# hanyas/mimo

Measured on AMD Instinct MI355X. Metric: E-step datapoint-component evals/sec, higher is better.
Workload: dtype f64

## Files before the change

include/mimo_hip.h:

```cpp
#ifndef MIMO_HIP_H
#define MIMO_HIP_H

#include <stddef.h>
#include <stdint.h>

#ifdef __cplusplus
extern "C" {
#endif

typedef struct mimo_ctx mimo_ctx;

#define MIMO_OK               0
#define MIMO_E_INVALID       -1
#define MIMO_E_HIP           -2
#define MIMO_E_NODATA        -3
#define MIMO_E_UNSUPPORTED   -4
#define MIMO_E_STATE         -5
#define MIMO_E_NOMEM         -6
#define MIMO_E_INTERNAL      -7

#define MIMO_F_KEEP_RESP      0x01
#define MIMO_F_KEEP_LOGP      0x02
#define MIMO_F_KEEP_LSE       0x04
#define MIMO_F_NO_STATS       0x08
// ... 155 lines not shown
                           const double* sx, const double* sn, const double* sxx,
                           double* alpha, double* qa, double* qb, double* qc, double* qd,
                           double* mus, double* psis, double* nus, double* half_logdet_psi, double* nat_c,
                           double* cc, double* bb, double* W, double* E2, double* E4, double* e_log_pi, double* c_total);
int mimo_host_gmm_vi_bound(int K, int D, int tied, const double* alpha0, const double* alpha, const double* e_log_pi,
                           const double* pa, const double* pb, const double* pc, const double* pd, const double* prior_logZ,
                           const double* qa, const double* qb, const double* qc, const double* qd,
                           const double* mus, const double* nus, const double* half_logdet_psi, const double* nat_c,
                           const double* bb, const double* E2, const double* W, const double* E4, double* vlb);

int mimo_host_block_order(int K, int D, const double* means, const double* mass, int block, int32_t* order);

int mimo_host_estep_certificate(int K, int D, const double* c0, const double* b0, const double* W0, const double* c, const double* b,
                                const double* W, double margin, double* out, double* table);

int mimo_host_legacy_draws(uint32_t* mt_key, int* mt_pos, int* has_gauss, double* gauss, int K, int n_before,
                           int n_gamma, int n_after, const double* shapes, double* before, double* gammas,
                           double* after);

int mimo_host_hier_vi(int K, int D, int nb_iter, const double* kap, const double* m0, double kappa0, const double* psi0_inv,
                      double nu0, const double* xk, const double* nk, const double* sxx_sum, double* mu_q, double* post_mus,
                      double* post_kappas, double* kappa_q, double* psi_q, double* nu_q);

int mimo_host_legacy_draws_inplace(uint32_t* mt_key, int* mt_pos, int has_gauss, double gauss, int K, int n_before,
                                   int n_gamma, int n_after, const double* shapes, double* before, double* gammas,
                                   double* after, int* redraw, uint32_t* final_state);

int mimo_host_py_sample(uint32_t* mt_key, int* mt_pos, int64_t n, int64_t k, int use_pool, int64_t* out);

int mimo_host_mnw_vi(int K, int dy, int dc, int affine, const double* a, const double* b, const double* c,
// ... 51 lines not shown
```

mimo_amd/_lib.py:

```python
import ctypes as C
import os
import sys

_HERE = os.path.dirname(os.path.abspath(__file__))
LIB_PATH = os.environ.get("MIMO_HIP_LIB") or os.path.join(_HERE, "libmimo_hip.so")

OK = 0
E_INVALID, E_HIP, E_NODATA, E_UNSUPPORTED, E_STATE, E_NOMEM, E_INTERNAL = -1, -2, -3, -4, -5, -6, -7
F_KEEP_RESP, F_KEEP_LOGP, F_KEEP_LSE, F_NO_STATS, F_DEVICE_OUT, F_DEVICE_IN, F_ENTROPY_SPLIT, F_ASYNC = 1, 2, 4, 8, 0x10, 0x20, 0x40, 0x80
F_WEIGHTS_RESIDENT = 0x100
F_DIAG_VAR = 0x200
F_SVI_RESIDENT_START = 0x400

_dp = C.POINTER(C.c_double)
_ip = C.POINTER(C.c_int32)
_vp = C.c_void_p

SIGNATURES = {
    "mimo_create": (C.c_int, [C.POINTER(_vp), C.c_int]),
    "mimo_destroy": (C.c_int, [_vp]),
    "mimo_last_error": (C.c_char_p, [_vp]),
    "mimo_set_stream": (C.c_int, [_vp, _vp]),
    "mimo_upload": (C.c_int, [_vp, _vp, C.c_int64, C.c_int]),
    "mimo_attach": (C.c_int, [_vp, _vp, C.c_int64, C.c_int]),
# ... 33 lines not shown
    "mimo_sample_from_log": (C.c_int, [_vp, _vp, C.c_int, C.c_int64, _vp, C.c_uint64, C.c_uint64, C.c_int, _vp, _vp]),
    "mimo_random_resp_stats": (C.c_int, [_vp, C.c_int, C.c_uint64, C.c_int, _vp]),
    "mimo_host_nw_vi": (C.c_int, [C.c_int, C.c_int] + [_vp] * 13),
    "mimo_host_nw_vi_tied": (C.c_int, [C.c_int, C.c_int] + [_vp] * 14),
    "mimo_host_nw_vlb": (C.c_int, [C.c_int, C.c_int] + [_vp] * 16),
    "mimo_host_legacy_draws_inplace": (C.c_int, [_vp, _vp, C.c_int, C.c_double, C.c_int, C.c_int, C.c_int, C.c_int,
                                                 _vp, _vp, _vp, _vp, C.POINTER(C.c_int), _vp]),
    "mimo_host_py_sample": (C.c_int, [_vp, C.POINTER(C.c_int), C.c_int64, C.c_int64, C.c_int, _vp]),
    "mimo_host_hier_vi": (C.c_int, [C.c_int, C.c_int, C.c_int, _vp, _vp, C.c_double, _vp, C.c_double] + [_vp] * 9),
    "mimo_host_legacy_draws": (C.c_int, [_vp, C.POINTER(C.c_int), C.POINTER(C.c_int), C.POINTER(C.c_double),
                                         C.c_int, C.c_int, C.c_int, C.c_int, _vp, _vp, _vp, _vp]),
    "mimo_host_gmm_vi_sweep": (C.c_int, [C.c_int, C.c_int, C.c_int] + [_vp] * 26),
    "mimo_host_gmm_vi_bound": (C.c_int, [C.c_int, C.c_int, C.c_int] + [_vp] * 21),
    "mimo_host_block_order": (C.c_int, [C.c_int, C.c_int, _vp, _vp, C.c_int, _vp]),
    "mimo_host_estep_certificate": (C.c_int, [C.c_int, C.c_int, _vp, _vp, _vp, _vp, _vp, _vp, C.c_double, _vp, _vp]),
    "mimo_host_mnw_vi": (C.c_int, [C.c_int, C.c_int, C.c_int, C.c_int] + [_vp] * 15),
    "mimo_host_nw_gibbs": (C.c_int, [C.c_int, C.c_int] + [_vp] * 10),
    "mimo_host_digamma": (C.c_double, [C.c_double]),
    "mimo_host_checksum": (C.c_int, [_vp, C.c_size_t, C.POINTER(C.c_uint64)]),
    "mimo_predict": (C.c_int, [_vp, _vp, _vp, _vp, C.c_int, _vp, _vp, _vp, C.c_int, C.c_int, C.c_int,
                               _vp, _vp, _vp, _vp, _vp, _vp]),
    "mimo_predict_flags": (C.c_int, [_vp, _vp, _vp, _vp, C.c_int, _vp, _vp, _vp, C.c_int, C.c_int, C.c_int,
                                     _vp, _vp, _vp, _vp, _vp, _vp, C.c_int]),
    "mimo_predict_batched": (C.c_int, [_vp, C.c_int, _vp, _vp, C.c_int64, C.c_int, _vp, _vp, _vp, _vp, C.c_int,
                                       _vp, _vp, _vp, C.c_int, C.c_int, _vp, _vp, _vp, _vp, _vp, _vp, _vp, C.c_int]),
    "mimo_get_resp": (C.c_int, [_vp, _vp]),
    "mimo_get_resp_columns": (C.c_int, [_vp, _vp, C.c_int64, _vp]),
    "mimo_get_logp": (C.c_int, [_vp, _vp]),
    "mimo_get_lse": (C.c_int, [_vp, _vp]),
    "mimo_get_labels": (C.c_int, [_vp, _vp]),
# ... 48 lines not shown
```

mimo_amd/csrc/mimo_abi.cpp:

```cpp
#include "mimo_abi_internal.h"
#include "mimo_kernels.h"
#include "mimo_extra.h"
#include "mimo_route.h"

#include <algorithm>
#include <cmath>
#include <cstdarg>
#include <cstdio>
#include <cstdlib>
#include <cstring>
#include <limits>
#include <new>
#include <stdexcept>
#include <string>
#include <vector>

using namespace mimo;
using namespace mimo_abi;

namespace mimo_comm {
int unique_id(char* out128, char* msg, size_t msglen);
int init(void** comm, const char* id128, int rank, int world, char* msg, size_t msglen);
int destroy(void* comm);
int allreduce_sum_f64(void* comm, double* buf, size_t count, hipStream_t stream, char* msg, size_t msglen);
// ... 109 lines not shown

static constexpr int kCertRenew = 16;
static constexpr double kCertEps = 1e-3;
static int cert_plan(mimo_ctx* ctx, const KernelArgs& a, const double* c, const double* b, const double* W, double* tab, int* kind) {
  *kind = kCertNone;
  const int K = a.K, D = ctx->D;
  if (!ctx->cert_on || a.resp_skip <= 0 || a.K16 != 4 || D < 14 || D > kMaxFusedD || ctx->structure != 0 || ctx->N < 1) return MIMO_OK;
  uint64_t part[4] = {0, 0, 0, 0};
  int32_t slot_of[64];
  for (int s = 0; s < K; ++s) { part[s >> 4] |= 1ull << ctx->order[s]; slot_of[ctx->order[s]] = s; }
  std::sort(part, part + 4);
  const bool stood = ctx->cert_prev_K == K && !memcmp(part, ctx->cert_prev_part, sizeof part);
  memcpy(ctx->cert_prev_part, part, sizeof part);
  ctx->cert_prev_K = K;
  if (ctx->cert_valid && (ctx->cert_K != K || ctx->cert_skip != a.resp_skip || memcmp(part, ctx->cert_part, sizeof part))) ctx->cert_valid = false;
  const size_t KD = (size_t)K * D, KDD = KD * D;
  if (ctx->cert_valid && ctx->cert_age < kCertRenew) {
    double out[5 * 64 + 4], t[4 + 2 * 64];
    const double* r = ctx->cert_ref.data();
    if (mimo_host_estep_certificate(K, D, r, r + K, r + K + KD, c, b, W, -0.6931471805599453 * a.resp_skip - kCertEps, out, t) == MIMO_OK) {
      memcpy(tab, t, 4 * sizeof(double));
      uint8_t* blk = reinterpret_cast<uint8_t*>(tab + 4 + 128);
      for (int s = 0; s < 64; ++s) {
        const int k = s < K ? ctx->cert_order[s] : -1;
        tab[4 + s] = k < 0 ? -1e300 : t[4 + k];
        tab[4 + 64 + s] = k < 0 ? 0.0 : t[4 + K + k];
        blk[s] = k < 0 ? 0 : (uint8_t)(slot_of[k] >> 4);
      }
      ctx->cert_age += 1;
      *kind = kCertCertified;
      return MIMO_OK;
    }
    ctx->cert_valid = false;
  }
  if (!stood) return MIMO_OK;
  int rc;
  if ((rc = ctx->cert_k.ensure(ctx, (size_t)ctx->N)) || (rc = ctx->cert_m.ensure(ctx, (size_t)ctx->N)) || (rc = ctx->cert_a.ensure(ctx, (size_t)ctx->N))) return rc;
  if (!ctx->cert_cnt.p) {
    if ((rc = ctx->cert_cnt.ensure(ctx, 4))) return rc;
    HIP_TRY(ctx, hipMemsetAsync(ctx->cert_cnt, 0, 4 * sizeof(unsigned long long), ctx->stream));
  }
  ctx->cert_ref.resize(K + KD + KDD);
  memcpy(ctx->cert_ref.data(), c, K * sizeof(double));
  memcpy(ctx->cert_ref.data() + K, b, KD * sizeof(double));
  memcpy(ctx->cert_ref.data() + K + KD, W, KDD * sizeof(double));
  memcpy(ctx->cert_order, ctx->order, K * sizeof(int32_t));
  memcpy(ctx->cert_part, part, sizeof part);
  ctx->cert_K = K; ctx->cert_skip = a.resp_skip; ctx->cert_age = 0;
  ctx->cert_valid = true;
  *kind = kCertReference;
  return MIMO_OK;
}

static void fill_args(mimo_ctx* ctx, int K, KernelArgs* a) {
  memset(a, 0, sizeof *a);
  a->Z = ctx->Z; a->N = ctx->N; a->D = ctx->D; a->K = K; a->K16 = (K + 15) / 16;
  a->F16 = ctx->F16;
  a->ZS = route_zs(K, ctx->D);
  a->RS = ctx->F16 + rs_pad();
  a->F16_total = ctx->F16;
// ... 1200 lines not shown
```

mimo_amd/csrc/mimo_host.cpp:

```cpp
#include <algorithm>
#include <atomic>
#include <condition_variable>
#include <functional>
#include <mutex>
#include <cmath>
#include <pthread.h>
#include <cstdint>
#include <cstdlib>
#include <cstring>
#include <new>
#include <stdexcept>
#include <system_error>
#include <thread>
#include <vector>

#include "../../include/mimo_hip.h"

namespace {

constexpr double kLog2Pi = 1.8378770664093454835606594728112;
constexpr double kLog2 = 0.69314718055994530941723212145818;

double digamma(double x) {
  double r = 0.0;
  while (x < 10.0) { r -= 1.0 / x; x += 1.0; }
  const double f = 1.0 / (x * x);
  const double t = f * (-1.0 / 12.0 + f * (1.0 / 120.0 + f * (-1.0 / 252.0 + f * (1.0 / 240.0 + f * (-1.0 / 132.0
                   + f * (691.0 / 32760.0 + f * (-1.0 / 12.0)))))));
// ... 967 lines not shown
    for (int i = c; i < A; ++i) {
      if (find(i) != c) continue;
      put(b >= 0 ? b : lightest(1), i);
    }
  }
  int s = 0;
  for (int k = 0; k < K; ++k) {
    if (mass[k] >= 1.0) continue;
    while (order[s] >= 0) ++s;
    order[s] = k;
  }
  return MIMO_OK;
  });
}

namespace {
constexpr double kCertGrid[] = {0.98, 0.95, 0.9, 0.8, 0.65, 0.5, 0.3, 0.1};

unsigned cert_chol4(v4d* __restrict__ M, int n) {
  unsigned bad = 0;
  v4d d0[32];
  for (int j = 0; j < n; ++j) d0[j] = M[j * n + j];
  for (int j = 0; j < n; ++j) {
    v4d* mj = M + (size_t)j * n;
    v4d d = mj[j], piv;
    for (int l = 0; l < 4; ++l) {
      if (!(d[l] > 1e-10 * std::fabs(d0[j][l]))) { bad |= 1u << l; d[l] = 1.0; }
      piv[l] = std::sqrt(d[l]);
    }
    const v4d inv = 1.0 / piv;
    for (int c = j; c < n; ++c) mj[c] *= inv;
    for (int i = j + 1; i < n; ++i) {
      const v4d f = mj[i];
      v4d* mi = M + (size_t)i * n;
      for (int c = i; c < n; ++c) mi[c] -= f * mj[c];
    }
  }
  return bad;
}
}

int mimo_host_estep_certificate(int K, int D, const double* c0, const double* b0, const double* W0, const double* c, const double* b,
                                const double* W, double margin, double* out, double* table) {
  return guarded_host([&]() -> int {
  if (K < 1 || D < 1 || !c0 || !b0 || !W0 || !c || !b || !W || !out) return MIMO_E_INVALID;
  if (K > 256 || D > 32) return MIMO_E_UNSUPPORTED;
  const size_t DD = (size_t)D * D;
  for (size_t i = 0; i < (size_t)K; ++i) if (!std::isfinite(c0[i]) || !std::isfinite(c[i])) return MIMO_E_INVALID;
  for (size_t i = 0; i < (size_t)K * D; ++i) if (!std::isfinite(b0[i]) || !std::isfinite(b[i])) return MIMO_E_INVALID;
  for (size_t i = 0; i < (size_t)K * DD; ++i) if (!std::isfinite(W0[i]) || !std::isfinite(W[i])) return MIMO_E_INVALID;
  double *ch0 = out, *ch = out + K, *rho = out + 2 * (size_t)K, *rhob = out + 3 * (size_t)K, *dk = out + 4 * (size_t)K, *cons = out + 5 * (size_t)K;
  std::vector<v4d> work(5 * DD);
  v4d *A0 = work.data(), *A1 = A0 + DD, *U0 = A1 + DD, *U1 = U0 + DD, *T = U1 + DD;
  v4d y[32], mu0[32], mu1[32];
  auto solve = [&](const v4d* U, const double* const rhs[4], v4d* mu) {
    v4d yy = {0.0, 0.0, 0.0, 0.0};
    for (int i = 0; i < D; ++i) {
      v4d s = {rhs[0][i], rhs[1][i], rhs[2][i], rhs[3][i]};
      for (int r = 0; r < i; ++r) s -= U[r * D + i] * y[r];
      y[i] = s / U[i * D + i];
      yy += y[i] * y[i];
    }
    for (int i = D - 1; i >= 0; --i) {
      v4d s = y[i];
      for (int r = i + 1; r < D; ++r) s -= U[i * D + r] * mu[r];
      mu[i] = s / U[i * D + i];
    }
    return yy;
  };
  for (int k0 = 0; k0 < K; k0 += 4) {
    int kk[4];
    for (int l = 0; l < 4; ++l) kk[l] = std::min(k0 + l, K - 1);
    const double *a0[4], *a1[4], *r0[4], *r1[4];
    for (int l = 0; l < 4; ++l) { a0[l] = W0 + kk[l] * DD; a1[l] = W + kk[l] * DD; r0[l] = b0 + (size_t)kk[l] * D; r1[l] = b + (size_t)kk[l] * D; }
    for (int i = 0; i < D; ++i)
      for (int j = i; j < D; ++j) {
        const size_t e = (size_t)i * D + j;
        U0[e] = A0[e] = v4d{a0[0][e], a0[1][e], a0[2][e], a0[3][e]};
        U1[e] = A1[e] = v4d{a1[0][e], a1[1][e], a1[2][e], a1[3][e]};
      }
    if (cert_chol4(U0, D) | cert_chol4(U1, D)) return MIMO_E_INVALID;
    const v4d q0 = solve(U0, r0, mu0), q1 = solve(U1, r1, mu1);
    v4d d2 = {0.0, 0.0, 0.0, 0.0};
    for (int i = 0; i < D; ++i) {
      v4d s = {0.0, 0.0, 0.0, 0.0};
      for (int r = i; r < D; ++r) s += U0[i * D + r] * (mu1[r] - mu0[r]);
      d2 += s * s;
    }
    unsigned same = 0;
    for (int l = 0; l < 4; ++l) if (!memcmp(a0[l], a1[l], DD * sizeof(double))) same |= 1u << l;
    double lo[4] = {0.0, 0.0, 0.0, 0.0}, hi[4] = {HUGE_VAL, HUGE_VAL, HUGE_VAL, HUGE_VAL};
    for (int side = 0; side < 2; ++side) {
      const v4d *P = side ? A0 : A1, *Q = side ? A1 : A0;
      unsigned pending = 0xFu & ~same;
      for (const double s : kCertGrid) {
        if (!pending) break;
        for (int i = 0; i < D; ++i)
          for (int j = i; j < D; ++j) T[i * D + j] = P[i * D + j] - s * Q[i * D + j];
        const unsigned ok = pending & ~cert_chol4(T, D);
        for (int l = 0; l < 4; ++l) if (ok >> l & 1u) { if (side) hi[l] = 1.0 / s; else lo[l] = s; }
        pending &= ~ok;
      }
    }
    for (int l = 0; l < 4 && k0 + l < K; ++l) {
      const int k = k0 + l;
      ch0[k] = c0[k] + 0.5 * q0[l];
      ch[k] = c[k] + 0.5 * q1[l];
      dk[k] = std::sqrt(d2[l]);
      rho[k] = (same >> l & 1u) ? 1.0 : lo[l];
      rhob[k] = (same >> l & 1u) ? 1.0 : hi[l];
    }
  }
  cons[0] = ch0[0]; cons[1] = ch[0]; cons[2] = rho[0]; cons[3] = dk[0];
  for (int k = 1; k < K; ++k) {
    cons[0] = std::min(cons[0], ch0[k]); cons[1] = std::max(cons[1], ch[k]);
    cons[2] = std::min(cons[2], rho[k]); cons[3] = std::max(cons[3], dk[k]);
  }
  if (!table) return MIMO_OK;
  std::vector<double> srt(ch0, ch0 + K);
  std::sort(srt.begin(), srt.end());
  double cut = HUGE_VAL, widest = 0.0;
// ... 11 lines not shown
    const double beta = rmin * (1.0 - e);
    table[2 * cl] = cmax - beta * c0min + 0.5 * rmin * (1.0 / e - 1.0) * dmax * dmax;
    table[2 * cl + 1] = beta;
  }
  double *gam = table + 4, *del = table + 4 + K;
  for (int k = 0; k < K; ++k) {
    if (!(rhob[k] < HUGE_VAL)) { gam[k] = -1e300; del[k] = 0.0; continue; }
    const double e = std::min(std::max(dk[k], 1e-12) / 4.0, 1.0);
    del[k] = rhob[k] * (1.0 + e);
    gam[k] = ch[k] - del[k] * ch0[k] - 0.5 * rhob[k] * (1.0 + 1.0 / e) * dk[k] * dk[k] + margin;
  }
  return MIMO_OK;
  });
}

double mimo_host_digamma(double x) { return digamma(x); }

int mimo_host_debug_fault(int kind) {
  return guarded_host([&]() -> int {
    if (kind == 1) throw std::bad_alloc();
    if (kind == 2) throw std::runtime_error("mimo_host_debug_fault");
    if (kind == 3) throw 42;
    if (kind == 4) { g_fail_thread_start.store(1); return MIMO_OK; }
    return kind == 0 ? MIMO_OK : MIMO_E_INVALID;
  });
}

}
```

mimo_amd/csrc/mimo_kernels.hip:

```cpp
#include "mimo_tile.h"
#include "mimo_extra.h"
#include <cstdio>
#include <cstdlib>

#include <math.h>
#include <type_traits>
#include <utility>

namespace mimo {

double philox_uniform_host(uint64_t seed, uint64_t row, uint64_t sweep) {
  return philox_uniform(seed, row, sweep);
}

#ifndef MIMO_ASYM_PRIO
#define MIMO_ASYM_PRIO 0
#endif
#define MFMA_PRIO()                                                                        \
  do {                                                                                    \
    if (MIMO_ASYM_PRIO && prio_hi) __builtin_amdgcn_s_setprio(1);                         \
    else __builtin_amdgcn_s_setprio(0);                                                   \
  } while (0)

#ifndef MIMO_STAGGER
// ... 144 lines not shown
    }
  };
  auto store_z = [&](int64_t t) {
#pragma unroll
    for (int i = 0; i < ZPT; ++i)
      if (zoff[i] >= 0) Zs[zoff[i]] = zr[i];
    if (tid < T) {
      if constexpr (TRIM) Zs[tid * ZS + D] = tid < clamp_scalar(N - t * T, T) ? 1.0 : 0.0;
      else Zs[tid * ZS + D] = (t * T + tid) < N ? 1.0 : 0.0;
      Zs[tid * ZS + D + 1] = 0.0;
    }
  };
  load_z(blockIdx.x);
  store_z(blockIdx.x);
  load_z((int64_t)blockIdx.x + gridDim.x);
  int ck = 0, nk = 0;
  double cm = 0.0, ca = 0.0, nm = 0.0, na = 0.0;
  auto load_cert = [&](int64_t t, int& k, double& m, double& av) {
    const int64_t n = t * T + (lane & 31);
    const bool in = n < N;
    k = in ? (int)a.cert_k[n] & 63 : 0;
    m = in ? a.cert_m[n] : 0.0;
    av = in ? a.cert_a[n] : 0.0;
  };
  double ctab[4] = {0.0, 0.0, 0.0, 0.0};
  double* const ctl = reinterpret_cast<double*>(fe + 2 * F16);
  uint32_t cnt_proven = 0, cnt_one = 0, cnt_all = 0;
  if constexpr (CERT == kCertCertified) {
    load_cert(blockIdx.x, ck, cm, ca);
    load_cert((int64_t)blockIdx.x + gridDim.x, nk, nm, na);
#pragma unroll
    for (int i = 0; i < 4; ++i) ctab[i] = a.cert_tab[i];
    for (int e = tid; e < kCertTabLen - 4; e += kWG) ctl[e] = a.cert_tab[4 + e];
  }

  const int frow = tid & (T - 1), fgrp = tid >> 5;
  wg_sync();
  uint32_t w[NCB];
  if constexpr (DS == 0) {
#pragma unroll
    for (int jj = 0; jj < NCB; ++jj) w[jj] = reinterpret_cast<const uint32_t*>(fe)[fgrp * NCB + jj];
  }

  STAGGER_START();
#ifdef MIMO_STAMPS
  unsigned long long st_sum[8] = {0, 0, 0, 0, 0, 0, 0, 0}, st_prev;
  asm volatile("s_memtime %0\n\ts_waitcnt lgkmcnt(0)" : "=s"(st_prev)::"memory");
#endif
#ifdef MIMO_STAMPS
  int st_it = 0;
#endif
  for (int64_t t = blockIdx.x; t < a.ntiles; t += gridDim.x) {
// ... 52 lines not shown
        const int k = kq + 8 * it;
        if (k < Kpad) Lt[pt * LS + k] = wv[it];
      }
    } else if constexpr (SRC == kSrcLabels) {
      if (tid < T) labs[tid] = (n0 + tid) < N ? a.labels[n0 + tid] : -1;
    }
    STAMP(1);
    MFMA_PRIO();
    wg_sync();
    STAMP(2);
#ifdef MIMO_STAMPS
    if (st_trace) st_tr[1] = st_prev;
#endif

    if constexpr (SRC == kSrcEstep) {
      uint32_t need = 0xFFFFFFFFu, computed = 0xFFFFFFFFu;
      if constexpr (CERT == kCertCertified) {
        const bool in = n0 + (lane & 31) < N;
        const double cgam = ctl[ck], cdel = ctl[64 + ck];
        const int cblk = reinterpret_cast<const uint8_t*>(ctl + 128)[ck];
        const double ub = fmax(fma(ctab[1], ca, ctab[0]), fma(ctab[3], ca, ctab[2]));
        const bool proven = in && ub <= fma(cdel, cm, cgam);
        const uint32_t pm = (uint32_t)__builtin_amdgcn_ballot_w64(proven);
        const uint32_t b0 = (uint32_t)__builtin_amdgcn_ballot_w64((cblk & 1) != 0), b1 = (uint32_t)__builtin_amdgcn_ballot_w64((cblk & 2) != 0);
        uint32_t eff[4];
#pragma unroll
        for (int w = 0; w < 4; ++w) {
          const uint32_t nd = ~pm | (((w & 1) ? b0 : ~b0) & ((w & 2) ? b1 : ~b1));
          eff[w] = __builtin_popcount(nd) <= 16 ? nd : 0xFFFFFFFFu;
        }
        need = wave == 0 ? eff[0] : wave == 1 ? eff[1] : wave == 2 ? eff[2] : eff[3];
        computed = lane < 16 ? eff[0] : lane < 32 ? eff[1] : lane < 48 ? eff[2] : eff[3];
        if (wave == 0) cnt_proven += __builtin_popcount(pm);
        cnt_one += need != 0xFFFFFFFFu ? 1u : 0u;
        cnt_all += 1u;
      }
      if constexpr (is_split) {
        if (sidx < 2) {
          gptr_t th = (gptr_t)(a.theta + (size_t)srb * NSI * 64);
          asm volatile("" : "+s"(th));
          const double* p = Ph + (16 * sidx + j) * RS + q;
          d4 acc = d4{0.0, 0.0, 0.0, 0.0};
          constexpr int PD = NS < 8 ? NS : 8;
          double tr[PD], bq[3];
#pragma unroll
          for (int e = 0; e < PD; ++e) tr[e] = th[e * 64 + lane];
          bq[0] = p[0];
          if (NS > 1) bq[1] = p[4];
#pragma unroll
          for (int s2 = 0; s2 < NS; ++s2) {
            if (s2 + 2 < NS) bq[(s2 + 2) % 3] = p[4 * (s2 + 2)];
// ... 3 lines not shown
            acc = __builtin_amdgcn_mfma_f64_16x16x4f64(av, bq[s2 % 3], acc, 0, 0, 0);
          }
          int lw_off = (16 * sidx + j) * LS + 16 * srb + q;
          asm volatile("" : "+v"(lw_off));
          double* lw = Lt + lw_off;
#pragma unroll
          for (int r = 0; r < 4; ++r) lw[4 * r] = acc[r];
        }
      } else if (wave < K16) {
        thw = thw0;
        asm volatile("" : "+s"(thw));
        if constexpr (SEED_TILE) load_seed(thw);
        const double* p0 = Ph + j * RS + q;
        const double* p1 = Ph + (16 + j) * RS + q;
        bool one_group = false;
        if constexpr (CERT == kCertCertified) one_group = need != 0xFFFFFFFFu;
        if (one_group) {
          if constexpr (CERT == kCertCertified) {
            const int cnt = __builtin_popcount(need);
            int rj = need ? __builtin_ctz(need) : 0;
            {
              uint32_t mleft = need;
              for (int jj = 0; mleft; ++jj) {
                rj = j == jj ? __builtin_ctz(mleft) : rj;
                mleft &= mleft - 1;
              }
            }
            int p_off = rj * RS + q;
            asm volatile("" : "+v"(p_off));
            const double* pc = Ph + p_off;
            d4 acc = SEED ? d4{cseed[0], cseed[1], cseed[2], cseed[3]} : d4{0.0, 0.0, 0.0, 0.0};
            double bq[3];
            bq[0] = pc[0];
            if (NS > 1) bq[1] = pc[4];
#pragma unroll
            for (int s = 0; s < NS; ++s) {
              if (s + 2 < NS) bq[(s + 2) % 3] = pc[4 * (s + 2)];
              __builtin_amdgcn_sched_barrier(0);
              const double av = ring[s % PF];
              ring[s % PF] = theta_slice((s + PF) % NEP);
              acc = __builtin_amdgcn_mfma_f64_16x16x4f64(av, bq[s % 3], acc, 0, 0, 0);
            }
            if (j < cnt) {
              int lw_off = rj * LS + 16 * wave + q;
              asm volatile("" : "+v"(lw_off));
              double* lw = Lt + lw_off;
#pragma unroll
              for (int r = 0; r < 4; ++r) lw[4 * r] = acc[r];
            }
          }
        } else {
#pragma unroll
        for (int h = 0; h < RBW / RP; ++h) {
          if (RBW == 1 || wave + 4 * h * RP < K16) {
            d4 acc[RP][2];
#pragma unroll
            for (int i2 = 0; i2 < RP; ++i2) {
              if constexpr (SEED) acc[i2][0] = acc[i2][1] = d4{cseed[0], cseed[1], cseed[2], cseed[3]};
              else { acc[i2][0] = d4{0.0, 0.0, 0.0, 0.0}; acc[i2][1] = d4{0.0, 0.0, 0.0, 0.0}; }
// ... 37 lines not shown
            }
          }
        }
        }
#pragma unroll
        for (int e = NE; e < NEP; ++e) ring[e % PF] = theta_slice((e + PF) % NEP);
      }
      STAMP(3);
      wg_sync();
      STAMP(4);

      __builtin_amdgcn_s_setprio(2);
      if constexpr (RBW == 1)
        normalise_tile<RBW, MODE, E2K, SKIP, LX, CERT>(a, Lt, LS, etab, K, K16, N, n0, wave, lane, gibbs, out_logp, out_resp,
                                                   out_lse, sc_lse, sc_rl, sc_prod, labs, pbatch, (int64_t)gridDim.x * T, lnt,
                                                   live, computed);
      else
        normalise_tile_chunked<RBW, MODE, LX>(a, Lt, LS, etab, K, K16, N, n0, wave, lane, gibbs, out_logp, out_resp,
                                          out_lse, sc_lse, sc_rl, sc_prod, labs, pbatch, (int64_t)gridDim.x * T);
      if constexpr (MODE != kGeneric) {
        if (++prod_tiles == 64) {
          sc_lse += log(sc_prod);
          sc_prod = 1.0;
          prod_tiles = 0;
        }
      }
      STAMP(5);
      MFMA_PRIO();
      wg_sync();
      STAMP(6);
    }
// ... 159 lines not shown
            bvq[cb] = pb[16 * cb];
            __builtin_amdgcn_sched_barrier(0);
          }
          avq = q < cnt ? avn : 0.0;
        }
#pragma unroll
        for (int cb = 0; cb < NCB; ++cb)
          sacc[0][cb] = __builtin_amdgcn_mfma_f64_16x16x4f64(avq, bvq[cb], sacc[0][cb], 0, 0, 0);
      };
      if constexpr (MODE == kFastGibbs || MODE == kModeLabels) stats_labels();
      else if constexpr (MODE == kGeneric) { if (gibbs) stats_labels(); else stats_nact(std::false_type{}); }
      else if constexpr (SKIP) stats_skip(__builtin_amdgcn_readfirstlane(live[wave]));
      else stats_nact(std::false_type{});
    }

    store_z(t + gridDim.x);
    load_z(t + 2 * (int64_t)gridDim.x);
    if constexpr (CERT == kCertCertified) {
      ck = nk; cm = nm; ca = na;
      load_cert(t + 2 * (int64_t)gridDim.x, nk, nm, na);
    }
    STAMP(7);
#ifdef MIMO_STAMPS
    if (st_trace) st_tr[3] = st_prev;
#endif
  }
#ifdef MIMO_STAMPS
  if (a.stamps && lane == 0)
    for (int i = 0; i < 8; ++i) a.stamps[((size_t)blockIdx.x * 4 + wave) * 8 + i] = st_sum[i];
#endif

  const int FT = a.F16_total;
  const size_t pstride = (size_t)Kpad * FT + 4;
  double* P = a.partials + (size_t)blockIdx.x * pstride + (SRC == kSrcEstep ? 0 : 16 * a.cb0);
  if constexpr (is_split) {
#pragma unroll
// ... 454 lines not shown
    else if (bb == D) Sk[1 + aa] = v;
    else { Sk[1 + D + aa * D + bb] = v; Sk[1 + D + bb * D + aa] = v; }
  }
  if (scalars && e == 0) {
    const double slse = red[(int64_t)Kpad * F16 + 0], srl = red[(int64_t)Kpad * F16 + 1];
    const bool split = red[(int64_t)Kpad * F16 + 2] > 0.0;
    scalars[0] = slse;
    const long long nan_bits = 0x7ff8000000000000LL;
    scalars[1] = __longlong_as_double(split ? __double_as_longlong(srl) : nan_bits);
    scalars[2] = __longlong_as_double(split ? __double_as_longlong(slse - srl) : nan_bits);
  }
}

size_t fused_lds_bytes(const KernelArgs& a, int src) {
  const bool e2k = src == kSrcEstep && !a.diag && a.D >= 14 && a.D <= kMaxFusedD && a.K16 <= 4;
  const size_t cert = src == kSrcEstep && a.cert == kCertCertified ? sizeof(double) * (kCertTabLen - 4) : 0;
  return sizeof(double) * ((size_t)kTile * (a.ZS + a.RS + a.LS) + 16 + (e2k ? kExpTab : 64)) + (size_t)a.F16 * 2 + cert;
}

static int rbw_for(int K16) { return K16 <= 4 ? 1 : 4; }
static int rbw_stats(int K16) { return K16 <= 4 ? 1 : K16 <= 8 ? 2 : 4; }

static int rbw_stats(int K16);

int stats_group_ncb(int K16) {
  static const int knob = [] { const char* e = getenv("MIMO_STATS_GROUP"); return e ? atoi(e) : 0; }();
  if (knob >= 1 && knob <= kMaxNCB && rbw_stats(K16) >= 2) return knob;
  return rbw_stats(K16) == 4 ? 5 : rbw_stats(K16) == 2 ? 6 : kMaxNCB;
}

bool fused_covers(int K16, int ncb, int src) {
// ... 254 lines not shown
```

mimo_amd/csrc/mimo_tile.h:

```cpp
#pragma once
#include "mimo_device.h"

#include <math.h>
#include <type_traits>
#include <utility>

namespace mimo {

#ifndef MIMO_EXP_CHAINS
#define MIMO_EXP_CHAINS 8
#endif

struct PhiloxBatch {
  double u = 0.0;
  int used = 8;
};
__device__ __forceinline__ double philox_for_tile(PhiloxBatch& pb, const KernelArgs& a, const int64_t n, const int lane,
                                                  const int64_t tile_stride_rows) {
  if (pb.used == 8) {
    pb.u = philox_uniform(a.seed, (uint64_t)(a.row0 + n + (int64_t)(lane >> 3) * tile_stride_rows), a.sweep);
    pb.used = 0;
  }
  const double uu = __shfl(pb.u, (pb.used << 3) | (lane & 7));
  pb.used += 1;
// ... 50 lines not shown
template <int MASK>
__device__ __forceinline__ void lane_xor_maxmin(double v, double& hi, double& lo) {
  const LanePair l = lane_xor_pair<MASK>(__double2loint(v)), h = lane_xor_pair<MASK>(__double2hiint(v));
  const double x = __hiloint2double(h.a, l.a), y = __hiloint2double(h.b, l.b);
  hi = fmax(x, y);
  lo = fmin(x, y);
}
template <int RBW, int MODE, bool E2K = false, bool SKIP = false, bool LX = false, int CERT = 0>
__device__ __forceinline__ void normalise_tile(const KernelArgs& a, double* __restrict__ Lt, const int LS,
                                               const double* __restrict__ etab, const int K, const int K16,
                                               const int64_t N, const int64_t n0, const int wave, const int lane,
                                               const bool gibbs, double* const out_logp, double* const out_resp,
                                               double* const out_lse, double& sc_lse, double& sc_rl, double& sc_prod,
                                               int* __restrict__ labs, PhiloxBatch& pb,
                                               const int64_t tstride, const double lnt = 0.0,
                                               uint32_t* __restrict__ live = nullptr, const uint32_t computed = 0) {
        static_assert(RBW == 1, "register variant: at most 8 components per lane");
        static_assert(!SKIP || MODE == kFastVI, "responsibility skip: softmax of the fast VI mode only");
        static_assert(CERT == 0 || (SKIP && LX), "certificates: the skipping softmax pass, lane exchanges in registers");
        const int pt = 8 * wave + (lane & 7), part = lane >> 3;
        const int CPP = 2 * K16, k0 = part * CPP;
        const int64_t n = n0 + pt;
        const bool valid = n < N;
        double* row = Lt + pt * LS + k0;

        auto body = [&](auto full_c) {
        constexpr bool FULL = decltype(full_c)::value;
        auto ok = [&](int c) { return FULL || c < CPP; };
        double x[8], lsave[8];
        if constexpr (CERT == kCertCertified && FULL) {
          const bool have = (computed >> pt) & 1u;
#pragma unroll
          for (int c = 0; c < 8; ++c) x[c] = have ? row[c] : -INFINITY;
        } else {
#pragma unroll
          for (int c = 0; c < 8; ++c) x[c] = ok(c) ? row[c] : -INFINITY;
        }
        if (out_logp && valid) {
#pragma unroll
          for (int c = 0; c < 8; ++c)
            if (c < CPP && k0 + c < K) out_logp[(int64_t)(k0 + c) * N + n] = x[c];
        }
        const double ml = tree_max8(x);
        double m = butterfly_max<LX, 8>(ml);
        if constexpr (CERT == kCertReference && FULL) {
          double m16, s16, s32, t32, u32;
          lane_xor_maxmin<16>(m, m16, s16);
          lane_xor_maxmin<32>(m16, m, t32);
// ... 313 lines not shown
```

Measured before the change: 136.5 billion.

## Precompute certificate reference factorisations and hoist per-tile skip descriptors ahead of tiles

```diff
diff --git a/include/mimo_hip.h b/include/mimo_hip.h
--- a/include/mimo_hip.h
+++ b/include/mimo_hip.h
@@ -193,6 +193,11 @@
 int mimo_host_estep_certificate(int K, int D, const double* c0, const double* b0, const double* W0, const double* c, const double* b,
                                 const double* W, double margin, double* out, double* table);
 
+size_t mimo_host_estep_certificate_ref_size(int K, int D);
+int mimo_host_estep_certificate_ref(int K, int D, const double* c0, const double* b0, const double* W0, double* ref);
+int mimo_host_estep_certificate_cur(int K, int D, const double* ref, const double* c, const double* b, const double* W, double margin,
+                                    double* out, double* table);
+
 int mimo_host_legacy_draws(uint32_t* mt_key, int* mt_pos, int* has_gauss, double* gauss, int K, int n_before,
                            int n_gamma, int n_after, const double* shapes, double* before, double* gammas,
                            double* after);
diff --git a/mimo_amd/_lib.py b/mimo_amd/_lib.py
--- a/mimo_amd/_lib.py
+++ b/mimo_amd/_lib.py
@@ -71,6 +71,9 @@
     "mimo_host_gmm_vi_bound": (C.c_int, [C.c_int, C.c_int, C.c_int] + [_vp] * 21),
     "mimo_host_block_order": (C.c_int, [C.c_int, C.c_int, _vp, _vp, C.c_int, _vp]),
     "mimo_host_estep_certificate": (C.c_int, [C.c_int, C.c_int, _vp, _vp, _vp, _vp, _vp, _vp, C.c_double, _vp, _vp]),
+    "mimo_host_estep_certificate_ref_size": (C.c_size_t, [C.c_int, C.c_int]),
+    "mimo_host_estep_certificate_ref": (C.c_int, [C.c_int, C.c_int, _vp, _vp, _vp, _vp]),
+    "mimo_host_estep_certificate_cur": (C.c_int, [C.c_int, C.c_int, _vp, _vp, _vp, _vp, C.c_double, _vp, _vp]),
     "mimo_host_mnw_vi": (C.c_int, [C.c_int, C.c_int, C.c_int, C.c_int] + [_vp] * 15),
     "mimo_host_nw_gibbs": (C.c_int, [C.c_int, C.c_int] + [_vp] * 10),
     "mimo_host_digamma": (C.c_double, [C.c_double]),
diff --git a/mimo_amd/csrc/mimo_abi.cpp b/mimo_amd/csrc/mimo_abi.cpp
--- a/mimo_amd/csrc/mimo_abi.cpp
+++ b/mimo_amd/csrc/mimo_abi.cpp
@@ -147,11 +147,9 @@
   memcpy(ctx->cert_prev_part, part, sizeof part);
   ctx->cert_prev_K = K;
   if (ctx->cert_valid && (ctx->cert_K != K || ctx->cert_skip != a.resp_skip || memcmp(part, ctx->cert_part, sizeof part))) ctx->cert_valid = false;
-  const size_t KD = (size_t)K * D, KDD = KD * D;
   if (ctx->cert_valid && ctx->cert_age < kCertRenew) {
     double out[5 * 64 + 4], t[4 + 2 * 64];
-    const double* r = ctx->cert_ref.data();
-    if (mimo_host_estep_certificate(K, D, r, r + K, r + K + KD, c, b, W, -0.6931471805599453 * a.resp_skip - kCertEps, out, t) == MIMO_OK) {
+    if (mimo_host_estep_certificate_cur(K, D, ctx->cert_ref.data(), c, b, W, -0.6931471805599453 * a.resp_skip - kCertEps, out, t) == MIMO_OK) {
       memcpy(tab, t, 4 * sizeof(double));
       uint8_t* blk = reinterpret_cast<uint8_t*>(tab + 4 + 128);
       for (int s = 0; s < 64; ++s) {
@@ -173,10 +171,8 @@
     if ((rc = ctx->cert_cnt.ensure(ctx, 4))) return rc;
     HIP_TRY(ctx, hipMemsetAsync(ctx->cert_cnt, 0, 4 * sizeof(unsigned long long), ctx->stream));
   }
-  ctx->cert_ref.resize(K + KD + KDD);
-  memcpy(ctx->cert_ref.data(), c, K * sizeof(double));
-  memcpy(ctx->cert_ref.data() + K, b, KD * sizeof(double));
-  memcpy(ctx->cert_ref.data() + K + KD, W, KDD * sizeof(double));
+  ctx->cert_ref.resize(mimo_host_estep_certificate_ref_size(K, D));
+  if ((rc = mimo_host_estep_certificate_ref(K, D, c, b, W, ctx->cert_ref.data())) != MIMO_OK && rc != MIMO_E_INVALID) return rc;
   memcpy(ctx->cert_order, ctx->order, K * sizeof(int32_t));
   memcpy(ctx->cert_part, part, sizeof part);
   ctx->cert_K = K; ctx->cert_skip = a.resp_skip; ctx->cert_age = 0;
diff --git a/mimo_amd/csrc/mimo_host.cpp b/mimo_amd/csrc/mimo_host.cpp
--- a/mimo_amd/csrc/mimo_host.cpp
+++ b/mimo_amd/csrc/mimo_host.cpp
@@ -12,6 +12,7 @@
 #include <stdexcept>
 #include <system_error>
 #include <thread>
+#include <memory>
 #include <vector>
 
 #include "../../include/mimo_hip.h"
@@ -1009,89 +1010,148 @@
   });
 }
 
+extern "C++" {
 namespace {
 constexpr double kCertGrid[] = {0.98, 0.95, 0.9, 0.8, 0.65, 0.5, 0.3, 0.1};
 
-unsigned cert_chol4(v4d* __restrict__ M, int n) {
+struct v4s { double v[4]; };
+inline v4d ld4(const v4d* p) { return *p; }
+inline v4d ld4(const v4s* p) { v4d r; memcpy(&r, p, sizeof r); return r; }
+inline void st4(v4d* p, v4d x) { *p = x; }
+inline void st4(v4s* p, v4d x) { memcpy(p, &x, sizeof x); }
+
+template <class V>
+unsigned cert_chol4(V* __restrict__ M, int n) {
   unsigned bad = 0;
   v4d d0[32];
-  for (int j = 0; j < n; ++j) d0[j] = M[j * n + j];
+  for (int j = 0; j < n; ++j) d0[j] = ld4(M + j * n + j);
   for (int j = 0; j < n; ++j) {
-    v4d* mj = M + (size_t)j * n;
-    v4d d = mj[j], piv;
+    V* mj = M + (size_t)j * n;
+    v4d d = ld4(mj + j), piv;
     for (int l = 0; l < 4; ++l) {
       if (!(d[l] > 1e-10 * std::fabs(d0[j][l]))) { bad |= 1u << l; d[l] = 1.0; }
       piv[l] = std::sqrt(d[l]);
     }
     const v4d inv = 1.0 / piv;
-    for (int c = j; c < n; ++c) mj[c] *= inv;
+    for (int c = j; c < n; ++c) st4(mj + c, ld4(mj + c) * inv);
     for (int i = j + 1; i < n; ++i) {
-      const v4d f = mj[i];
-      v4d* mi = M + (size_t)i * n;
-      for (int c = i; c < n; ++c) mi[c] -= f * mj[c];
+      const v4d f = ld4(mj + i);
+      V* mi = M + (size_t)i * n;
+      for (int c = i; c < n; ++c) st4(mi + c, ld4(mi + c) - f * ld4(mj + c));
     }
   }
   return bad;
 }
-}
-
-int mimo_host_estep_certificate(int K, int D, const double* c0, const double* b0, const double* W0, const double* c, const double* b,
-                                const double* W, double margin, double* out, double* table) {
-  return guarded_host([&]() -> int {
-  if (K < 1 || D < 1 || !c0 || !b0 || !W0 || !c || !b || !W || !out) return MIMO_E_INVALID;
+
+template <class VU, class VM>
+v4d cert_solve4(const VU* U, const double* const rhs[4], VM* mu, v4d* y, int D) {
+  v4d yy = {0.0, 0.0, 0.0, 0.0};
+  for (int i = 0; i < D; ++i) {
+    v4d s = {rhs[0][i], rhs[1][i], rhs[2][i], rhs[3][i]};
+    for (int r = 0; r < i; ++r) s -= ld4(U + r * D + i) * y[r];
+    y[i] = s / ld4(U + i * D + i);
+    yy += y[i] * y[i];
+  }
+  for (int i = D - 1; i >= 0; --i) {
+    v4d s = y[i];
+    for (int r = i + 1; r < D; ++r) s -= ld4(U + i * D + r) * ld4(mu + r);
+    st4(mu + i, s / ld4(U + i * D + i));
+  }
+  return yy;
+}
+}
+}
+
+namespace {
+constexpr size_t kCertRefHead = 4;
+inline size_t cert_ref_group(int D) { return (2 * (size_t)D * D + D) * 4; }
+}
+
+size_t mimo_host_estep_certificate_ref_size(int K, int D) {
+  if (K < 1 || D < 1 || K > 256 || D > 32) return 0;
+  return kCertRefHead + (size_t)K + (size_t)((K + 3) / 4) * cert_ref_group(D);
+}
+
+int mimo_host_estep_certificate_ref(int K, int D, const double* c0, const double* b0, const double* W0, double* ref) {
+  return guarded_host([&]() -> int {
+  if (K < 1 || D < 1 || !c0 || !b0 || !W0 || !ref) return MIMO_E_INVALID;
   if (K > 256 || D > 32) return MIMO_E_UNSUPPORTED;
   const size_t DD = (size_t)D * D;
-  for (size_t i = 0; i < (size_t)K; ++i) if (!std::isfinite(c0[i]) || !std::isfinite(c[i])) return MIMO_E_INVALID;
-  for (size_t i = 0; i < (size_t)K * D; ++i) if (!std::isfinite(b0[i]) || !std::isfinite(b[i])) return MIMO_E_INVALID;
-  for (size_t i = 0; i < (size_t)K * DD; ++i) if (!std::isfinite(W0[i]) || !std::isfinite(W[i])) return MIMO_E_INVALID;
-  double *ch0 = out, *ch = out + K, *rho = out + 2 * (size_t)K, *rhob = out + 3 * (size_t)K, *dk = out + 4 * (size_t)K, *cons = out + 5 * (size_t)K;
-  std::vector<v4d> work(5 * DD);
-  v4d *A0 = work.data(), *A1 = A0 + DD, *U0 = A1 + DD, *U1 = U0 + DD, *T = U1 + DD;
-  v4d y[32], mu0[32], mu1[32];
-  auto solve = [&](const v4d* U, const double* const rhs[4], v4d* mu) {
-    v4d yy = {0.0, 0.0, 0.0, 0.0};
-    for (int i = 0; i < D; ++i) {
-      v4d s = {rhs[0][i], rhs[1][i], rhs[2][i], rhs[3][i]};
-      for (int r = 0; r < i; ++r) s -= U[r * D + i] * y[r];
-      y[i] = s / U[i * D + i];
-      yy += y[i] * y[i];
-    }
-    for (int i = D - 1; i >= 0; --i) {
-      v4d s = y[i];
-      for (int r = i + 1; r < D; ++r) s -= U[i * D + r] * mu[r];
-      mu[i] = s / U[i * D + i];
-    }
-    return yy;
-  };
-  for (int k0 = 0; k0 < K; k0 += 4) {
+  ref[0] = K; ref[1] = D; ref[2] = -1.0; ref[3] = 0.0;
+  for (size_t i = 0; i < (size_t)K; ++i) if (!std::isfinite(c0[i])) return MIMO_E_INVALID;
+  for (size_t i = 0; i < (size_t)K * D; ++i) if (!std::isfinite(b0[i])) return MIMO_E_INVALID;
+  for (size_t i = 0; i < (size_t)K * DD; ++i) if (!std::isfinite(W0[i])) return MIMO_E_INVALID;
+  double* ch0 = ref + kCertRefHead;
+  double* grp = ch0 + K;
+  v4d y[32];
+  int g = 0;
+  for (int k0 = 0; k0 < K; k0 += 4, ++g, grp += cert_ref_group(D)) {
     int kk[4];
     for (int l = 0; l < 4; ++l) kk[l] = std::min(k0 + l, K - 1);
-    const double *a0[4], *a1[4], *r0[4], *r1[4];
-    for (int l = 0; l < 4; ++l) { a0[l] = W0 + kk[l] * DD; a1[l] = W + kk[l] * DD; r0[l] = b0 + (size_t)kk[l] * D; r1[l] = b + (size_t)kk[l] * D; }
+    const double *a0[4], *r0[4];
+    for (int l = 0; l < 4; ++l) { a0[l] = W0 + kk[l] * DD; r0[l] = b0 + (size_t)kk[l] * D; }
+    v4s *A0 = reinterpret_cast<v4s*>(grp), *U0 = A0 + DD, *mu0 = U0 + DD;
+    for (size_t e = 0; e < DD; ++e) U0[e] = A0[e] = v4s{{a0[0][e], a0[1][e], a0[2][e], a0[3][e]}};
+    ref[2] = g;
+    if (cert_chol4(U0, D)) return MIMO_E_INVALID;
+    const v4d q0 = cert_solve4(U0, r0, mu0, y, D);
+    for (int l = 0; l < 4 && k0 + l < K; ++l) ch0[k0 + l] = c0[k0 + l] + 0.5 * q0[l];
+  }
+  ref[2] = g;
+  return MIMO_OK;
+  });
+}
+
+int mimo_host_estep_certificate_cur(int K, int D, const double* ref, const double* c, const double* b, const double* W, double margin,
+                                    double* out, double* table) {
+  return guarded_host([&]() -> int {
+  if (K < 1 || D < 1 || !ref || !c || !b || !W || !out) return MIMO_E_INVALID;
+  if (K > 256 || D > 32) return MIMO_E_UNSUPPORTED;
+  if (ref[0] != (double)K || ref[1] != (double)D) return MIMO_E_INVALID;
+  const size_t DD = (size_t)D * D;
+  if (ref[2] < 0.0) return MIMO_E_INVALID;
+  for (size_t i = 0; i < (size_t)K; ++i) if (!std::isfinite(c[i])) return MIMO_E_INVALID;
+  for (size_t i = 0; i < (size_t)K * D; ++i) if (!std::isfinite(b[i])) return MIMO_E_INVALID;
+  for (size_t i = 0; i < (size_t)K * DD; ++i) if (!std::isfinite(W[i])) return MIMO_E_INVALID;
+  const int good = (int)ref[2];
+  const double *rch0 = ref + kCertRefHead, *grp = rch0 + K;
+  double *ch0 = out, *ch = out + K, *rho = out + 2 * (size_t)K, *rhob = out + 3 * (size_t)K, *dk = out + 4 * (size_t)K, *cons = out + 5 * (size_t)K;
+  std::vector<v4d> work(3 * DD);
+  v4d *A1 = work.data(), *U1 = A1 + DD, *T = U1 + DD;
+  v4d y[32], mu1[32];
+  int g = 0;
+  for (int k0 = 0; k0 < K; k0 += 4, ++g, grp += cert_ref_group(D)) {
+    int kk[4];
+    for (int l = 0; l < 4; ++l) kk[l] = std::min(k0 + l, K - 1);
+    const double *a1[4], *r1[4];
+    for (int l = 0; l < 4; ++l) { a1[l] = W + kk[l] * DD; r1[l] = b + (size_t)kk[l] * D; }
+    const v4s *A0 = reinterpret_cast<const v4s*>(grp), *U0 = A0 + DD, *mu0 = U0 + DD;
     for (int i = 0; i < D; ++i)
       for (int j = i; j < D; ++j) {
         const size_t e = (size_t)i * D + j;
-        U0[e] = A0[e] = v4d{a0[0][e], a0[1][e], a0[2][e], a0[3][e]};
         U1[e] = A1[e] = v4d{a1[0][e], a1[1][e], a1[2][e], a1[3][e]};
       }
-    if (cert_chol4(U0, D) | cert_chol4(U1, D)) return MIMO_E_INVALID;
-    const v4d q0 = solve(U0, r0, mu0), q1 = solve(U1, r1, mu1);
+    if ((g >= good) | (cert_chol4(U1, D) != 0)) return MIMO_E_INVALID;
+    const v4d q1 = cert_solve4(U1, r1, mu1, y, D);
     v4d d2 = {0.0, 0.0, 0.0, 0.0};
     for (int i = 0; i < D; ++i) {
       v4d s = {0.0, 0.0, 0.0, 0.0};
-      for (int r = i; r < D; ++r) s += U0[i * D + r] * (mu1[r] - mu0[r]);
+      for (int r = i; r < D; ++r) s += ld4(U0 + i * D + r) * (mu1[r] - ld4(mu0 + r));
       d2 += s * s;
     }
     unsigned same = 0;
-    for (int l = 0; l < 4; ++l) if (!memcmp(a0[l], a1[l], DD * sizeof(double))) same |= 1u << l;
+    for (int l = 0; l < 4; ++l) {
+      size_t e = 0;
+      while (e < DD && !memcmp(&A0[e].v[l], a1[l] + e, sizeof(double))) ++e;
+      if (e == DD) same |= 1u << l;
+    }
     double lo[4] = {0.0, 0.0, 0.0, 0.0}, hi[4] = {HUGE_VAL, HUGE_VAL, HUGE_VAL, HUGE_VAL};
     for (int side = 0; side < 2; ++side) {
-      const v4d *P = side ? A0 : A1, *Q = side ? A1 : A0;
       unsigned pending = 0xFu & ~same;
       for (const double s : kCertGrid) {
         if (!pending) break;
         for (int i = 0; i < D; ++i)
-          for (int j = i; j < D; ++j) T[i * D + j] = P[i * D + j] - s * Q[i * D + j];
+          for (int j = i; j < D; ++j) T[i * D + j] = side ? ld4(A0 + i * D + j) - s * A1[i * D + j] : A1[i * D + j] - s * ld4(A0 + i * D + j);
         const unsigned ok = pending & ~cert_chol4(T, D);
         for (int l = 0; l < 4; ++l) if (ok >> l & 1u) { if (side) hi[l] = 1.0 / s; else lo[l] = s; }
         pending &= ~ok;
@@ -1099,7 +1159,7 @@
     }
     for (int l = 0; l < 4 && k0 + l < K; ++l) {
       const int k = k0 + l;
-      ch0[k] = c0[k] + 0.5 * q0[l];
+      ch0[k] = rch0[k];
       ch[k] = c[k] + 0.5 * q1[l];
       dk[k] = std::sqrt(d2[l]);
       rho[k] = (same >> l & 1u) ? 1.0 : lo[l];
@@ -1141,6 +1201,19 @@
   });
 }
 
+
+int mimo_host_estep_certificate(int K, int D, const double* c0, const double* b0, const double* W0, const double* c, const double* b,
+                                const double* W, double margin, double* out, double* table) {
+  return guarded_host([&]() -> int {
+  if (K < 1 || D < 1 || !c0 || !b0 || !W0 || !c || !b || !W || !out) return MIMO_E_INVALID;
+  if (K > 256 || D > 32) return MIMO_E_UNSUPPORTED;
+  const std::unique_ptr<double[]> ref(new double[mimo_host_estep_certificate_ref_size(K, D)]);
+  const int rc = mimo_host_estep_certificate_ref(K, D, c0, b0, W0, ref.get());
+  if (rc != MIMO_OK && rc != MIMO_E_INVALID) return rc;
+  return mimo_host_estep_certificate_cur(K, D, ref.get(), c, b, W, margin, out, table);
+  });
+}
+
 double mimo_host_digamma(double x) { return digamma(x); }
 
 int mimo_host_debug_fault(int kind) {
diff --git a/mimo_amd/csrc/mimo_kernels.hip b/mimo_amd/csrc/mimo_kernels.hip
--- a/mimo_amd/csrc/mimo_kernels.hip
+++ b/mimo_amd/csrc/mimo_kernels.hip
@@ -182,8 +182,8 @@
   load_z(blockIdx.x);
   store_z(blockIdx.x);
   load_z((int64_t)blockIdx.x + gridDim.x);
-  int ck = 0, nk = 0;
-  double cm = 0.0, ca = 0.0, nm = 0.0, na = 0.0;
+  int nk = 0;
+  double nm = 0.0, na = 0.0;
   auto load_cert = [&](int64_t t, int& k, double& m, double& av) {
     const int64_t n = t * T + (lane & 31);
     const bool in = n < N;
@@ -193,17 +193,50 @@
   };
   double ctab[4] = {0.0, 0.0, 0.0, 0.0};
   double* const ctl = reinterpret_cast<double*>(fe + 2 * F16);
+  double* const ninf = ctl + (kCertTabLen - 4);
   uint32_t cnt_proven = 0, cnt_one = 0, cnt_all = 0;
+  uint32_t d_need = 0xFFFFFFFFu;
+  int d_poff = 0, d_lwoff = 0, d_roff = 0;
+  auto cert_descriptor = [&](int64_t t, int k, double m, double av) {
+    if (t >= a.ntiles) return;
+    const bool in = t * T + (lane & 31) < N;
+    const double cgam = ctl[k], cdel = ctl[64 + k];
+    const int cblk = reinterpret_cast<const uint8_t*>(ctl + 128)[k];
+    const double ub = fmax(fma(ctab[1], av, ctab[0]), fma(ctab[3], av, ctab[2]));
+    const bool proven = in && ub <= fma(cdel, m, cgam);
+    const uint32_t pm = (uint32_t)__builtin_amdgcn_ballot_w64(proven);
+    const uint32_t b0 = (uint32_t)__builtin_amdgcn_ballot_w64((cblk & 1) != 0), b1 = (uint32_t)__builtin_amdgcn_ballot_w64((cblk & 2) != 0);
+    auto dead = [&](int w) -> uint32_t { return pm & ((b0 ^ (0u - (w & 1))) | (b1 ^ (0u - ((w >> 1) & 1)))); };
+    const uint32_t dw = dead(wave);
+    d_need = __builtin_popcount(dw) >= 16 ? ~dw : 0xFFFFFFFFu;
+    const uint32_t dl = dead(lane >> 4);
+    const int pt = 8 * wave + (lane & 7);
+    const bool have = __builtin_popcount(dl) < 16 || !((dl >> pt) & 1u);
+    d_roff = have ? pt * LS + 8 * (lane >> 3) : (int)(ninf - Lt);
+    const int rank = __builtin_amdgcn_mbcnt_lo(d_need, 0);
+    const bool push = lane < 32 && ((d_need >> (lane & 31)) & 1u);
+    const int got = __builtin_amdgcn_ds_permute((push ? rank : 63) << 2, lane);
+    const int rj = __builtin_amdgcn_ds_bpermute(j << 2, got) & 31;
+    d_poff = rj * RS + q;
+    d_lwoff = rj * LS + 16 * wave + q;
+    if (wave == 0) cnt_proven += __builtin_popcount(pm);
+    cnt_one += d_need != 0xFFFFFFFFu ? 1u : 0u;
+    cnt_all += 1u;
+  };
   if constexpr (CERT == kCertCertified) {
-    load_cert(blockIdx.x, ck, cm, ca);
-    load_cert((int64_t)blockIdx.x + gridDim.x, nk, nm, na);
+    load_cert(blockIdx.x, nk, nm, na);
 #pragma unroll
     for (int i = 0; i < 4; ++i) ctab[i] = a.cert_tab[i];
     for (int e = tid; e < kCertTabLen - 4; e += kWG) ctl[e] = a.cert_tab[4 + e];
+    if (tid < 8) ninf[tid] = -INFINITY;
   }
 
   const int frow = tid & (T - 1), fgrp = tid >> 5;
   wg_sync();
+  if constexpr (CERT == kCertCertified) {
+    cert_descriptor(blockIdx.x, nk, nm, na);
+    load_cert((int64_t)blockIdx.x + gridDim.x, nk, nm, na);
+  }
   uint32_t w[NCB];
   if constexpr (DS == 0) {
 #pragma unroll
@@ -286,27 +319,6 @@
 #endif
 
     if constexpr (SRC == kSrcEstep) {
-      uint32_t need = 0xFFFFFFFFu, computed = 0xFFFFFFFFu;
-      if constexpr (CERT == kCertCertified) {
-        const bool in = n0 + (lane & 31) < N;
-        const double cgam = ctl[ck], cdel = ctl[64 + ck];
-        const int cblk = reinterpret_cast<const uint8_t*>(ctl + 128)[ck];
-        const double ub = fmax(fma(ctab[1], ca, ctab[0]), fma(ctab[3], ca, ctab[2]));
-        const bool proven = in && ub <= fma(cdel, cm, cgam);
-        const uint32_t pm = (uint32_t)__builtin_amdgcn_ballot_w64(proven);
-        const uint32_t b0 = (uint32_t)__builtin_amdgcn_ballot_w64((cblk & 1) != 0), b1 = (uint32_t)__builtin_amdgcn_ballot_w64((cblk & 2) != 0);
-        uint32_t eff[4];
-#pragma unroll
-        for (int w = 0; w < 4; ++w) {
-          const uint32_t nd = ~pm | (((w & 1) ? b0 : ~b0) & ((w & 2) ? b1 : ~b1));
-          eff[w] = __builtin_popcount(nd) <= 16 ? nd : 0xFFFFFFFFu;
-        }
-        need = wave == 0 ? eff[0] : wave == 1 ? eff[1] : wave == 2 ? eff[2] : eff[3];
-        computed = lane < 16 ? eff[0] : lane < 32 ? eff[1] : lane < 48 ? eff[2] : eff[3];
-        if (wave == 0) cnt_proven += __builtin_popcount(pm);
-        cnt_one += need != 0xFFFFFFFFu ? 1u : 0u;
-        cnt_all += 1u;
-      }
       if constexpr (is_split) {
         if (sidx < 2) {
           gptr_t th = (gptr_t)(a.theta + (size_t)srb * NSI * 64);
@@ -340,19 +352,11 @@
         const double* p0 = Ph + j * RS + q;
         const double* p1 = Ph + (16 + j) * RS + q;
         bool one_group = false;
-        if constexpr (CERT == kCertCertified) one_group = need != 0xFFFFFFFFu;
+        if constexpr (CERT == kCertCertified) one_group = d_need != 0xFFFFFFFFu;
         if (one_group) {
           if constexpr (CERT == kCertCertified) {
-            const int cnt = __builtin_popcount(need);
-            int rj = need ? __builtin_ctz(need) : 0;
-            {
-              uint32_t mleft = need;
-              for (int jj = 0; mleft; ++jj) {
-                rj = j == jj ? __builtin_ctz(mleft) : rj;
-                mleft &= mleft - 1;
-              }
-            }
-            int p_off = rj * RS + q;
+            const int cnt = __builtin_popcount(d_need);
+            int p_off = d_poff;
             asm volatile("" : "+v"(p_off));
             const double* pc = Ph + p_off;
             d4 acc = SEED ? d4{cseed[0], cseed[1], cseed[2], cseed[3]} : d4{0.0, 0.0, 0.0, 0.0};
@@ -368,7 +372,7 @@
               acc = __builtin_amdgcn_mfma_f64_16x16x4f64(av, bq[s % 3], acc, 0, 0, 0);
             }
             if (j < cnt) {
-              int lw_off = rj * LS + 16 * wave + q;
+              int lw_off = d_lwoff;
               asm volatile("" : "+v"(lw_off));
               double* lw = Lt + lw_off;
 #pragma unroll
@@ -436,7 +440,7 @@
       if constexpr (RBW == 1)
         normalise_tile<RBW, MODE, E2K, SKIP, LX, CERT>(a, Lt, LS, etab, K, K16, N, n0, wave, lane, gibbs, out_logp, out_resp,
                                                    out_lse, sc_lse, sc_rl, sc_prod, labs, pbatch, (int64_t)gridDim.x * T, lnt,
-                                                   live, computed);
+                                                   live, d_roff);
       else
         normalise_tile_chunked<RBW, MODE, LX>(a, Lt, LS, etab, K, K16, N, n0, wave, lane, gibbs, out_logp, out_resp,
                                           out_lse, sc_lse, sc_rl, sc_prod, labs, pbatch, (int64_t)gridDim.x * T);
@@ -626,12 +630,12 @@
       else stats_nact(std::false_type{});
     }
 
+    if constexpr (CERT == kCertCertified) {
+      cert_descriptor(t + gridDim.x, nk, nm, na);
+      load_cert(t + 2 * (int64_t)gridDim.x, nk, nm, na);
+    }
     store_z(t + gridDim.x);
     load_z(t + 2 * (int64_t)gridDim.x);
-    if constexpr (CERT == kCertCertified) {
-      ck = nk; cm = nm; ca = na;
-      load_cert(t + 2 * (int64_t)gridDim.x, nk, nm, na);
-    }
     STAMP(7);
 #ifdef MIMO_STAMPS
     if (st_trace) st_tr[3] = st_prev;
@@ -1116,7 +1120,7 @@
 
 size_t fused_lds_bytes(const KernelArgs& a, int src) {
   const bool e2k = src == kSrcEstep && !a.diag && a.D >= 14 && a.D <= kMaxFusedD && a.K16 <= 4;
-  const size_t cert = src == kSrcEstep && a.cert == kCertCertified ? sizeof(double) * (kCertTabLen - 4) : 0;
+  const size_t cert = src == kSrcEstep && a.cert == kCertCertified ? sizeof(double) * (kCertTabLen - 4 + 8) : 0;
   return sizeof(double) * ((size_t)kTile * (a.ZS + a.RS + a.LS) + 16 + (e2k ? kExpTab : 64)) + (size_t)a.F16 * 2 + cert;
 }
 
diff --git a/mimo_amd/csrc/mimo_tile.h b/mimo_amd/csrc/mimo_tile.h
--- a/mimo_amd/csrc/mimo_tile.h
+++ b/mimo_amd/csrc/mimo_tile.h
@@ -88,7 +88,7 @@
                                                double* const out_lse, double& sc_lse, double& sc_rl, double& sc_prod,
                                                int* __restrict__ labs, PhiloxBatch& pb,
                                                const int64_t tstride, const double lnt = 0.0,
-                                               uint32_t* __restrict__ live = nullptr, const uint32_t computed = 0) {
+                                               uint32_t* __restrict__ live = nullptr, const int cert_row = 0) {
         static_assert(RBW == 1, "register variant: at most 8 components per lane");
         static_assert(!SKIP || MODE == kFastVI, "responsibility skip: softmax of the fast VI mode only");
         static_assert(CERT == 0 || (SKIP && LX), "certificates: the skipping softmax pass, lane exchanges in registers");
@@ -103,9 +103,9 @@
         auto ok = [&](int c) { return FULL || c < CPP; };
         double x[8], lsave[8];
         if constexpr (CERT == kCertCertified && FULL) {
-          const bool have = (computed >> pt) & 1u;
-#pragma unroll
-          for (int c = 0; c < 8; ++c) x[c] = have ? row[c] : -INFINITY;
+          const double* src = Lt + cert_row;
+#pragma unroll
+          for (int c = 0; c < 8; ++c) x[c] = src[c];
         } else {
 #pragma unroll
           for (int c = 0; c < 8; ++c) x[c] = ok(c) ? row[c] : -INFINITY;
```

Measured after the change: 148.0 billion, median of 6. 1.08x the previous value.
